# castorini/dhr

Hardware: AMD Instinct MI355X
Metric: queries/sec (exact top-1000, brute-force dense-hybrid GIP retrieval) (higher is better)
Workload: dtype i8 (bound GEMM: gated AND ungated columns int8 x int8 -> int32 on the matrix cores, every gated rounding upward, the ungated quantisation error paid by the filter margin) + f64-accumulated f16 x f32 exact rescoring of the survivors -- the returned scores are the exact scores rounded once, identical

## Files before the change

dhr_amd/csrc/dhr_internal.h:

```cpp
#pragma once
#include <hip/hip_runtime.h>
#include <hip/hip_fp16.h>
#include <stdint.h>

#include "../../include/dhr_hip.h"
#include "abi_guard.h"

extern "C" int dhr_set_error_message(int code, const char* msg);
extern "C" int dhr_index_device(const dhr_index* ix);
extern "C" void dhr_internal_index_arena(dhr_index* ix, void*** base, size_t** bytes);
extern "C" int dhr_internal_search_begin_async(dhr_index* ix, const dhr_query_batch* qb, int32_t k, float* out_sample_scores_dev, void* stream);
extern "C" void dhr_internal_search_abort(dhr_index* ix);
extern "C" int dhr_internal_search_pre_async(dhr_index* ix, const dhr_query_batch* qb, int32_t k, int32_t r_local, float* out_scores_dev, void* stream);
extern "C" int dhr_internal_search_begin_rest_async(dhr_index* ix, const float* tau_dev, float* out_sample_scores_dev, void* stream);
extern "C" int dhr_internal_search_mid_async(dhr_index* ix, const float* tau_hat_dev, int32_t r_local, float* out_scores_dev, void* stream);
extern "C" int dhr_internal_search_finish_async(dhr_index* ix, const float* tau_hat_dev, float* out_scores, int64_t* out_rows, int32_t* out_count_dev,
                                                int32_t out_mem_kind, void* stream);

namespace dhr {

constexpr int TILE_ROWS = 256;
constexpr int TILE_K = 64;
constexpr int CHUNK = 8;
constexpr int TILE_HALVES = TILE_ROWS * TILE_K;
constexpr int SP_A_BYTES = 16384;
constexpr int SP_IDX_BYTES = 2048;
constexpr int SP_STAGE_A = SP_A_BYTES + SP_IDX_BYTES;
constexpr int SP_STAGE_B = 16384;
constexpr int SP_DENSE = 16384;
constexpr int SP_SLOT = SP_STAGE_A + SP_STAGE_B;
constexpr int S8_A_BYTES = 8192;
constexpr int S8_STAGE_A = S8_A_BYTES + 2048;
#ifndef DHR_HEAVY
#define DHR_HEAVY 64
#endif
constexpr int HEAVY = DHR_HEAVY;
constexpr int HEAVY_KEY_STRIDE = HEAVY * 6 / 4;
constexpr int HEAVY_VAL_STRIDE = HEAVY * 6 / 2;
#ifndef DHR_DOC_GROUP
#define DHR_DOC_GROUP 4
#endif
constexpr int DOC_GROUP = DHR_DOC_GROUP;

__host__ __device__ inline int64_t tiled_chunk_offset(int64_t row, int chunk, int ksteps) {
  const int64_t tile = row >> 8;
  const int rl = (int)(row & 255);
  const int ks = chunk >> 3, cc = chunk & 7;
  const int phys = cc ^ ((rl >> 1) & 7);
  return ((tile * ksteps + ks) * TILE_ROWS + rl) * (int64_t)TILE_K + phys * CHUNK;
}

__host__ __device__ inline uint32_t f32_ordered(float f) {
  union { float f; uint32_t u; } v; v.f = f;
  if ((v.u << 1) == 0u) return 0x80000000u;
  return (v.u & 0x80000000u) ? ~v.u : (v.u | 0x80000000u);
}
__host__ __device__ inline float ordered_f32(uint32_t o) {
  union { float f; uint32_t u; } v;
  v.u = (o & 0x80000000u) ? (o & 0x7FFFFFFFu) : ~o;
  return v.f;
}
__host__ __device__ inline int64_t seq_to_tile(int64_t i, int map_mode, int period, int64_t head, int64_t perm_mul = 1, int64_t perm_n = 1) {
  if (map_mode == 0) return i;
  if (map_mode == 1) return head + i * period;
  if (map_mode == 3) i = (i * perm_mul) % perm_n;
  return head + (i / (period - 1)) * period + i % (period - 1) + 1;
}
__host__ __device__ inline int64_t divmod24(int64_t x, int64_t n, double inv_n, int64_t& rem) {
  const double xd = (double)(int32_t)(x >> 24) * 16777216.0 + (double)(int32_t)(x & 0xFFFFFF);
  int64_t q = (int64_t)(int32_t)(xd * inv_n);
  int64_t r = x - q * n;
  if (r < 0) { r += n; --q; } else if (r >= n) { r -= n; ++q; }
  rem = r;
  return q;
}
__host__ __device__ inline int64_t seq_to_tile_fast(int64_t i, int map_mode, int period, int64_t head, int64_t perm_mul, int64_t perm_n,
                                                    double inv_perm_n, double inv_pm1) {
  if (map_mode == 0) return i;
  if (map_mode == 1) return head + i * period;
  if (map_mode == 3) (void)divmod24(i * perm_mul, perm_n, inv_perm_n, i);
  int64_t rem;
  const int64_t q = divmod24(i, period - 1, inv_pm1, rem);
  return head + q * period + rem + 1;
}
__host__ __device__ inline uint64_t make_key(float score, uint32_t row) {
  return ((uint64_t)f32_ordered(score) << 32) | (uint64_t)(0xFFFFFFFFu - row);
}

struct GemmArgs {
  const __half* a_tiles;
  const __half* b_tiles;
  int ksteps;
  int k_split;
  int ts, td;
  int ts_q;
  int64_t seq_lo, seq_hi;
  int map_mode, period;
  int64_t perm_mul, perm_n;
  double inv_perm_n, inv_pm1;
  int64_t head, n_tiles;
  int n_qtiles;
  int64_t n_rows;
  const float* thr;
  uint2* cand;
  uint32_t* cnt;
  uint32_t cap;
  float* dump;
  int64_t dump_ld;
  int64_t dump_row0;
  int n_queries;
  int variant;
  const int32_t* g8_shift;
  const int32_t* g8_rsum;
  int partial_wn;
  uint32_t* p_ctr;
  int64_t p_groups;
  const float* i8_mul;
  const struct ListTier* tier;
};
struct ListTier { uint2* ovf; const uint32_t* ovf_off; const uint32_t* ovf_cap; };
#if defined(__HIPCC__)
// ... 204 lines not shown
```

dhr_amd/csrc/index_build.hip:

```cpp
#include <fcntl.h>
#include <sys/mman.h>
#include <sys/stat.h>
#include <unistd.h>

#include "dhr_state.h"

extern "C" void dhr_index_destroy(dhr_index* ix) try {
  if (!ix) return;
  hipSetDevice(ix->device);
  free_ws(ix->ws);
  free_ws(ix->ws_fb[0]);
  free_ws(ix->ws_fb[1]);
  if (ix->s_aux) hipStreamDestroy(ix->s_aux);
  if (ix->s_gemm) hipStreamDestroy(ix->s_gemm);
  hipFree(ix->sh_arena);
  hipFree(ix->resid8); hipFree(ix->i8_col_scale); hipFree(ix->g8_inv_cs); hipFree(ix->g8_w); hipFree(ix->g8_rsum); hipFree(ix->tiles); hipFree(ix->c_idx); hipFree(ix->vals_rm); hipFree(ix->bucket_map); hipFree(ix->heavy_key);
  delete ix;
} DHR_CATCH_VOID

static int g_opt_dense_i8 = -1;
static int g_opt_gated_i8 = -1;
constexpr int64_t GATED_I8_MIN_ROWS = 1000000, GATED_I8_MIN_ROWS_NARROW = 4000000;
constexpr int64_t DENSE_ONLY_I8_MIN_ROWS = 1000000;
extern "C" int dhr_set_option(int32_t option, int64_t value) try {
// ... 274 lines not shown
        ix->i8_scale = ix->i8_ec = ix->i8_nc = 0.f;
        ix->td = ((d->d_cls + 31) / 32 + 1) & ~1;
        ix->kt = ix->td * 32;
        ix->ksteps = (ix->kt + TILE_K - 1) / TILE_K;
      }
    }
  }
  {
    const int ld = (int)round_up(ix->d_cls, 256) / 2;
    if (ix->dense_i8 && ix->d_dlr == 0 && ld <= 512 && ix->i8_ec > 0.f) {
      const size_t rb = (size_t)ix->n_rows * ld;
      if (hipMalloc((void**)&ix->resid8, rb) != hipSuccess) return fail(set_error(DHR_ERR_HIP, "hipMalloc of the residual image failed"));
      ix->index_bytes += (int64_t)rb;
      ix->resid_ld = ld;
      if (launch_resid_build(ix->vals_rm, ix->k_rm, ix->n_rows, ix->d_dlr, ix->d_cls, ix->i8_col_scale, ix->resid8, ld, s) != hipSuccess)
        return fail(set_error(DHR_ERR_HIP, "residual image launch failed"));
      ix->resid_ec2 = std::sqrt((float)ix->d_cls) * ix->i8_scale / 28.f;
    }
  }
  const size_t tile_bytes = (size_t)ix->n_tiles * ((size_t)ix->ts * (ix->gated_i8 ? S8_STAGE_A : SP_STAGE_A) + (size_t)ix->td * SP_DENSE);
  if (hipMalloc((void**)&ix->tiles, tile_bytes) != hipSuccess)
    return fail(set_error(DHR_ERR_HIP, "hipMalloc of " + std::to_string(tile_bytes) + " bytes for the corpus tiles failed"));
  ix->index_bytes += (int64_t)tile_bytes;
  if (ix->gated_i8) {
    float gmax;
    memcpy(&gmax, &flags[3], 4);
    std::vector<uint32_t> cm((size_t)ix->d_dlr, 0u);
    {
      DevMem cmd;
      uint32_t*& d_cm = (uint32_t*&)cmd.p;
      if (hipMalloc((void**)&d_cm, cm.size() * 4) != hipSuccess || hipMalloc((void**)&ix->g8_inv_cs, cm.size() * 4) != hipSuccess ||
          hipMalloc((void**)&ix->g8_w, cm.size() * 4) != hipSuccess)
        return fail(set_error(DHR_ERR_HIP, "hipMalloc failed"));
      if (hipMemsetAsync(d_cm, 0, cm.size() * 4, s) != hipSuccess ||
          launch_col_absmax(ix->vals_rm, ix->k_rm, ix->n_rows, 0, ix->d_dlr, d_cm, s) != hipSuccess ||
          hipMemcpy(cm.data(), d_cm, cm.size() * 4, hipMemcpyDeviceToHost) != hipSuccess)
        return fail(set_error(DHR_ERR_HIP, "column scan failed"));
    }
    ix->g8_sref = (gmax > 0.f ? gmax : 1.f) * (1.00001f / 127.f);
    std::vector<float> inv(cm.size()), wj(cm.size());
    for (size_t j = 0; j < cm.size(); ++j) {
      float m;
      memcpy(&m, &cm[j], 4);
      const float ratio = m > 0.f ? std::min(m / gmax, 1.f) : 1.f;
      const float f = std::max(std::pow(ratio, 0.75f), 1.f / 1024.f);
      inv[j] = 1.000001f / (ix->g8_sref * f);
      wj[j] = f * 1.000001f;
    }
    if (hipMemcpy(ix->g8_inv_cs, inv.data(), inv.size() * 4, hipMemcpyHostToDevice) != hipSuccess ||
        hipMemcpy(ix->g8_w, wj.data(), wj.size() * 4, hipMemcpyHostToDevice) != hipSuccess)
      return fail(set_error(DHR_ERR_HIP, "hipMemcpy failed"));
    ix->g8_max_shift = 0;
    while (ix->g8_max_shift < 7 && 255.0 * 127.0 * (double)(ix->ts * 32) * (double)(2 << ix->g8_max_shift) <= 1073741824.0) ++ix->g8_max_shift;
    const size_t rb = (size_t)ix->n_tiles * TILE_ROWS * 4;
    if (hipMalloc((void**)&ix->g8_rsum, rb) != hipSuccess) return fail(set_error(DHR_ERR_HIP, "hipMalloc failed"));
    ix->index_bytes += (int64_t)rb;
    if (launch_g8_row_sum(ix->vals_rm, ix->k_rm, ix->n_rows, ix->n_tiles * TILE_ROWS, ix->d_dlr, ix->abs_mode, ix->g8_inv_cs, ix->g8_rsum, s) != hipSuccess)
      return fail(set_error(DHR_ERR_HIP, "g8_row_sum launch failed"));
  }
  if (has_idx && ix->n_buckets == 1) {
    const size_t mb = (size_t)d->d_dlr * 256;
    if (hipMalloc((void**)&ix->bucket_map, mb) != hipSuccess || hipMemsetAsync(ix->bucket_map, 0, mb, s) != hipSuccess)
      return fail(set_error(DHR_ERR_HIP, "bucket map allocation failed"));
  }
  if (has_idx && ix->n_buckets > 1 && idx_esize(d->index_dtype) == 1) {
    const size_t hb = (size_t)d->d_dlr * 256 * 4;
    if (hipMalloc((void**)&d_hist, hb) != hipSuccess || hipMemsetAsync(d_hist, 0, hb, s) != hipSuccess)
      return fail(set_error(DHR_ERR_HIP, "hipMalloc (index histogram) failed"));
    if (launch_idx_hist((const uint8_t*)ix->c_idx, ix->vals_rm, ix->k_rm, d->n_rows, d->d_dlr, (float*)d_hist, s) != hipSuccess)
      return fail(set_error(DHR_ERR_HIP, "idx_hist launch failed"));
    std::vector<float> hist((size_t)d->d_dlr * 256);
    if (hipMemcpy(hist.data(), d_hist, hb, hipMemcpyDeviceToHost) != hipSuccess) return fail(set_error(DHR_ERR_HIP, "hipMemcpy failed"));
    std::vector<uint8_t> map;
    build_bucket_map(hist, d->d_dlr, ix->n_buckets, map);
    if (hipMalloc((void**)&ix->bucket_map, map.size()) != hipSuccess ||
        hipMemcpy(ix->bucket_map, map.data(), map.size(), hipMemcpyHostToDevice) != hipSuccess)
      return fail(set_error(DHR_ERR_HIP, "bucket map upload failed"));
  }
  if ((rc = build_tiles(ix, s)) != DHR_OK) return fail(rc);
  if (has_idx && d->d_dlr <= 4096) {
    const size_t hb = (size_t)d->n_rows * HEAVY_KEY_STRIDE * 4;
    if (hipMalloc((void**)&ix->heavy_key, hb) != hipSuccess)
      return fail(set_error(DHR_ERR_HIP, "hipMalloc of the refine lists failed"));
    ix->heavy_val = (__half*)((char*)ix->heavy_key + HEAVY * 4);
    ix->index_bytes += (int64_t)hb;
    if (launch_heavy_build(ix->vals_rm, ix->k_rm, ix->c_idx, ix->idx_dtype, d->n_rows, d->d_dlr, ix->bucket_map, ix->n_buckets,
                           ix->heavy_key, ix->heavy_val, ix->gated_i8 ? ix->g8_inv_cs : nullptr, ix->abs_mode ? 1 : 0, s) != hipSuccess)
      return fail(set_error(DHR_ERR_HIP, "heavy_build launch failed"));
  }
  if (hipStreamSynchronize(s) != hipSuccess) return fail(set_error(DHR_ERR_HIP, "index build failed on the device"));
  build.ix = nullptr;
  *out = ix;
  return DHR_OK;
} DHR_CATCH_STATUS

namespace {
struct FileHeader {
  char magic[8];
  uint32_t version, header_bytes;
  int64_t n_rows, row_offset;
  int32_t d_dlr, d_cls, k_rm, idx_dtype, idx_buckets, pad0;
  uint64_t val_offset, val_bytes, idx_offset, idx_bytes, blob_offset, blob_bytes;
};
static_assert(sizeof(FileHeader) <= 4096, "header must fit one page");
const char FILE_MAGIC[8] = {'D', 'H', 'R', 'I', 'D', 'X', '1', 0};
constexpr uint32_t FILE_VERSION = 1;

bool write_all(int fd, const void* p, size_t n) {
  const char* c = (const char*)p;
  while (n) {
    const ssize_t w = write(fd, c, n);
    if (w <= 0) return false;
    c += w; n -= (size_t)w;
  }
  return true;
}
int read_header(const char* path, FileHeader& h, int* fd_out) {
  if (!path) return set_error(DHR_ERR_INVALID, "null path");
  const int fd = open(path, O_RDONLY);
  if (fd < 0) return set_error(DHR_ERR_INVALID, std::string("cannot open ") + path);
  char page[4096];
  const ssize_t got = pread(fd, page, sizeof(page), 0);
  if (got != (ssize_t)sizeof(page)) { close(fd); return set_error(DHR_ERR_INVALID, std::string(path) + " is not a device-ready index file (short header)"); }
  memcpy(&h, page, sizeof(h));
  if (memcmp(h.magic, FILE_MAGIC, 8) != 0 || h.header_bytes != 4096) { close(fd); return set_error(DHR_ERR_INVALID, std::string(path) + " is not a device-ready index file"); }
  if (h.version != FILE_VERSION) {
    close(fd);
    return set_error(DHR_ERR_UNSUPPORTED, std::string(path) + " has file format version " + std::to_string(h.version) + ", this library reads version " +
                                          std::to_string(FILE_VERSION));
  }
  if (fd_out) *fd_out = fd; else close(fd);
  return DHR_OK;
}
}

extern "C" int dhr_index_save(const dhr_index* ix, const char* path, const void* blob, int64_t blob_bytes) try {
  if (!ix || !path || blob_bytes < 0 || (blob_bytes > 0 && !blob)) return set_error(DHR_ERR_INVALID, "null index / path or bad blob");
  HIP_TRY(hipSetDevice(ix->device));
  FileHeader h{};
  memcpy(h.magic, FILE_MAGIC, 8);
  h.version = FILE_VERSION; h.header_bytes = 4096;
  h.n_rows = ix->n_rows; h.row_offset = ix->row_offset;
  h.d_dlr = ix->d_dlr; h.d_cls = ix->d_cls; h.k_rm = ix->k_rm; h.idx_dtype = ix->idx_dtype; h.idx_buckets = ix->idx_buckets_req;
  h.pad0 = ix->dlr_pad;
  h.val_offset = 4096; h.val_bytes = (uint64_t)ix->n_rows * ix->k_rm * 2;
  h.idx_offset = (h.val_offset + h.val_bytes + 4095) / 4096 * 4096;
  h.idx_bytes = ix->c_idx ? (uint64_t)ix->n_rows * ix->d_dlr * idx_esize(ix->idx_dtype) : 0;
  h.blob_offset = (h.idx_offset + h.idx_bytes + 4095) / 4096 * 4096;
  h.blob_bytes = (uint64_t)blob_bytes;
  const int fd = open(path, O_WRONLY | O_CREAT | O_TRUNC, 0644);
  if (fd < 0) return set_error(DHR_ERR_INVALID, std::string("cannot create ") + path);
  const size_t CH = (size_t)64 << 20;
  void* pin = nullptr;
  if (hipHostMalloc(&pin, CH, hipHostMallocDefault) != hipSuccess) { close(fd); return set_error(DHR_ERR_HIP, "hipHostMalloc failed"); }
  auto fail = [&](int code) { hipHostFree(pin); close(fd); unlink(path); return code; };
  char page[4096] = {0};
  memcpy(page, &h, sizeof(h));
  if (!write_all(fd, page, 4096)) return fail(set_error(DHR_ERR_INVALID, "write failed (header)"));
  const void* src[2] = {ix->vals_rm, ix->c_idx};
  const uint64_t off[2] = {h.val_offset, h.idx_offset}, bytes[2] = {h.val_bytes, h.idx_bytes};
  for (int i = 0; i < 2; ++i) {
    if (lseek(fd, (off_t)off[i], SEEK_SET) < 0) return fail(set_error(DHR_ERR_INVALID, "seek failed"));
    for (uint64_t done = 0; done < bytes[i]; done += CH) {
      const size_t n = (size_t)std::min<uint64_t>(CH, bytes[i] - done);
      if (hipMemcpy(pin, (const char*)src[i] + done, n, hipMemcpyDeviceToHost) != hipSuccess) return fail(set_error(DHR_ERR_HIP, "D2H copy failed while saving"));
      if (!write_all(fd, pin, n)) return fail(set_error(DHR_ERR_INVALID, "write failed (disk full?)"));
    }
// ... 54 lines not shown
```

dhr_amd/csrc/kernels.hip:

```cpp
#include <algorithm>
#include <cstdlib>
#include <mutex>

#include "dhr_internal.h"
#include "gemm_common.h"
#include <type_traits>

namespace dhr {

typedef short short8 __attribute__((ext_vector_type(8)));

static hipError_t ensure_lds_attr(const void* fn, int bytes, int (&have)[64]) {
  static std::mutex mu;
  int dev = 0;
  (void)hipGetDevice(&dev);
  std::lock_guard<std::mutex> lock(mu);
  if (bytes <= have[dev & 63]) return hipSuccess;
  const hipError_t e = hipFuncSetAttribute(fn, hipFuncAttributeMaxDynamicSharedMemorySize, bytes);
  if (e == hipSuccess) have[dev & 63] = bytes;
  return e;
}

__device__ __forceinline__ float wave_sum(float v) {
#pragma unroll
// ... 668 lines not shown
  __syncthreads();
  for (int d = 512; d > 0; d >>= 1) {
    if (tid < d) part[tid] += part[tid + d];
    __syncthreads();
  }
  if (tid == 0) {
    const unsigned long long total = part[0] + 256ull * (unsigned long long)n_queries;
    scale_s = total > arena_entries ? (double)arena_entries / (double)total : 1.0;
  }
  __syncthreads();
  const double scale = scale_s;
  auto seg = [&](int q) -> uint32_t {
    const uint32_t w = want(q);
    if (w == 0u) return 0u;
    const uint32_t v = scale < 1.0 ? (uint32_t)((double)w * scale) : w;
    return (v + 255u) & ~255u;
  };
  __syncthreads();
  s = 0;
  for (int q = lo; q < hi; ++q) s += seg(q);
  part[tid] = s;
  __syncthreads();
  for (int d = 1; d < 1024; d <<= 1) {
    const unsigned long long v = tid >= d ? part[tid - d] : 0ull;
    __syncthreads();
    part[tid] += v;
    __syncthreads();
  }
  unsigned long long run = tid ? part[tid - 1] : 0ull;
  for (int q = lo; q < hi; ++q) {
    uint32_t w = seg(q);
    if (run >= arena_entries) w = 0u;
    else if (run + w > arena_entries) w = (uint32_t)(arena_entries - run);
    ovf_off[q] = (uint32_t)(run < arena_entries ? run : arena_entries);
    ovf_cap[q] = w;
    run += seg(q);
  }
}
hipError_t launch_plan_overflow(const uint32_t* cnt_prev, double rows_ratio, uint32_t cap, uint32_t max_extra, uint32_t arena_entries, int n_queries,
                                uint32_t* ovf_off, uint32_t* ovf_cap, hipStream_t s) {
  hipLaunchKernelGGL(plan_overflow_kernel, dim3(1), dim3(1024), 0, s, cnt_prev, rows_ratio, cap, max_extra, arena_entries, n_queries, ovf_off, ovf_cap);
  return hipGetLastError();
}
__device__ __forceinline__ bool flat_block(const uint32_t* __restrict__ offs, int n_queries, uint32_t b, int& q, uint32_t& blk) {
  if (b >= offs[n_queries]) return false;
  int lo = 0, hi = n_queries;
  while (hi - lo > 1) {
    const int mid = (lo + hi) >> 1;
    if (offs[mid] <= b) lo = mid; else hi = mid;
  }
  q = lo; blk = b - offs[lo];
  return true;
}

template <int SL>
__global__ void __launch_bounds__(256) heavy_build_kernel(const __half* __restrict__ vals_rm, int k_rm,
                                                          const void* __restrict__ idx, int idx_dtype, int64_t n_rows,
                                                          int d_dlr, const uint8_t* __restrict__ map, int n_buckets,
                                                          uint32_t* __restrict__ heavy_key, __half* __restrict__ heavy_val,
                                                          const float* __restrict__ g8_inv_cs, int abs_mode) {
  const int lane = threadIdx.x & 63;
  const int64_t wave0 = (int64_t)blockIdx.x * 4 + (threadIdx.x >> 6);
  const int64_t nwaves = (int64_t)gridDim.x * 4;
  for (int64_t row = wave0; row < n_rows; row += nwaves) {
    constexpr int MAXJ = 64 * SL - 1;
    uint32_t key[SL];
#pragma unroll
    for (int sl = 0; sl < SL; ++sl) {
      const int j = lane + 64 * sl;
      key[sl] = 0u;
      if (j < d_dlr) {
        union { _Float16 h; uint16_t u; } cv; cv.h = (_Float16)__half2float(vals_rm[row * k_rm + j]);
        const uint32_t mag = cv.u & 0x7FFFu;
        if (mag) key[sl] = (mag << 16) | (uint32_t)(MAXJ - j);
      }
    }
    for (int r = 0; r < HEAVY; ++r) {
      uint32_t best = 0u;
#pragma unroll
      for (int sl = 0; sl < SL; ++sl) best = key[sl] > best ? key[sl] : best;
#pragma unroll
      for (int o = 32; o > 0; o >>= 1) { const uint32_t ob = __shfl_xor(best, o, 64); best = ob > best ? ob : best; }
      if (best == 0u) {
        if (lane == 0) for (int rr = r; rr < HEAVY; ++rr) { heavy_key[row * HEAVY_KEY_STRIDE + rr] = 0xFFFFFFFFu; heavy_val[row * HEAVY_VAL_STRIDE + rr] = __float2half(0.f); }
        break;
      }
      const int j = MAXJ - (int)(best & 0xFFFFu);
      if ((j & 63) == lane) {
        const int iv = load_idx(idx, idx_dtype, row * d_dlr + j);
        const uint32_t bk = n_buckets > 1 ? (uint32_t)bucket_of(iv, j, map, n_buckets) : 0u;
        uint32_t key_out = ((uint32_t)j << 20) | (bk << 16) | ((uint32_t)iv & 0xFFFFu);
        if (g8_inv_cs) {
          float d = __half2float(vals_rm[row * k_rm + j]);
          if (abs_mode) d = fabsf(d);
          const uint32_t lvl = d > 0.f ? (uint32_t)quant_up_i8(d, g8_inv_cs[j]) : 0u;
          key_out = ((uint32_t)j << 20) | ((lvl >> 4) << 17) | ((bk & 1u) << 16) | ((lvl & 0xFu) << 12) | ((uint32_t)iv & 0xFFFu);
        }
        heavy_key[row * HEAVY_KEY_STRIDE + r] = key_out;
        heavy_val[row * HEAVY_VAL_STRIDE + r] = vals_rm[row * k_rm + j];
#pragma unroll
        for (int sl = 0; sl < SL; ++sl) if (sl == (j >> 6)) key[sl] = 0u;
      }
    }
  }
}
hipError_t launch_heavy_build(const __half* vals_rm, int k_rm, const void* idx, int idx_dtype, int64_t n_rows, int d_dlr,
                              const uint8_t* map, int n_buckets, uint32_t* heavy_key, __half* heavy_val, const float* g8_inv_cs, int abs_mode, hipStream_t s) {
  if (n_rows <= 0) return hipSuccess;
  const int64_t blocks = (n_rows + 3) / 4;
  if (d_dlr <= 1024)
    hipLaunchKernelGGL(heavy_build_kernel<16>, dim3((unsigned)(blocks < 16384 ? blocks : 16384)), dim3(256), 0, s, vals_rm, k_rm,
                       idx, idx_dtype, n_rows, d_dlr, map, n_buckets, heavy_key, heavy_val, g8_inv_cs, abs_mode);
  else
    hipLaunchKernelGGL(heavy_build_kernel<64>, dim3((unsigned)(blocks < 16384 ? blocks : 16384)), dim3(256), 0, s, vals_rm, k_rm,
                       idx, idx_dtype, n_rows, d_dlr, map, n_buckets, heavy_key, heavy_val, g8_inv_cs, abs_mode);
  return hipGetLastError();
}

static __device__ __forceinline__ uint4 gather16(const void* p) { return *(const uint4*)p; }
static __device__ __forceinline__ uint2 gather8(const void* p) { return *(const uint2*)p; }
#ifndef REFINE_PREFETCH
#define REFINE_PREFETCH 2
#endif
#ifndef REFINE_WPE
#define REFINE_WPE 8
#endif
#if REFINE_WPE > 0
#define REFINE_ATTR __attribute__((amdgpu_waves_per_eu(REFINE_WPE)))
#else
#define REFINE_ATTR
#endif
template <bool G8>
__global__ void __launch_bounds__(256) REFINE_ATTR refine_kernel(RefineArgs p) {
  extern __shared__ uint32_t qw[];
  int q = blockIdx.y;
  uint32_t blk = blockIdx.x;
  for (uint32_t fb = blockIdx.x;; fb += gridDim.x) {
  if (p.blk_off && !flat_block(p.blk_off, p.n_queries, fb, q, blk)) return;
  uint32_t count = p.cnt[q];
  const uint32_t cap_q = p.ovf_cap ? p.cap + p.ovf_cap[q] : p.cap;
  if (count > cap_q) count = cap_q;
  const uint32_t base = blk * REFINE_PER_WG;
  if (base >= count) { if (p.blk_off) continue; return; }
  __syncthreads();
  for (int j = threadIdx.x; j < p.d_dlr; j += 256) {
    if constexpr (G8) { qw[2 * j] = p.q_pack[(int64_t)q * p.d_dlr + j]; qw[2 * j + 1] = p.g8_q8[(int64_t)q * p.d_dlr + j]; }
    else qw[j] = p.q_pack[(int64_t)q * p.d_dlr + j];
  }
  __syncthreads();
  const int sub = threadIdx.x & 7;
  const float t = p.thr[q];
  const double unit = G8 ? (double)p.g8_unit[q] : 0.0;
  auto entry = [&](uint32_t i) __attribute__((always_inline)) -> uint2 {
    if (i >= count || i >= base + REFINE_PER_WG) return make_uint2(0u, 0u);
    return i < p.cap ? p.cand[(int64_t)q * p.cap + i] : p.ovf[(size_t)p.ovf_off[q] + (i - p.cap)];
  };
  constexpr int EPL = HEAVY / 8;
  static_assert(EPL == 8 || EPL == 4, "8 lanes per candidate read 8 or 4 entries each");
  struct Rec { uint4 k0, k1, hv; };
  auto record = [&](uint32_t i, const uint2 c, Rec& r) __attribute__((always_inline)) {
    r.k0 = r.k1 = make_uint4(0xFFFFFFFFu, 0xFFFFFFFFu, 0xFFFFFFFFu, 0xFFFFFFFFu);
    r.hv = make_uint4(0u, 0u, 0u, 0u);
    if (i < count && i < base + REFINE_PER_WG) {
      const uint32_t* hk = p.heavy_key + (int64_t)c.x * HEAVY_KEY_STRIDE + sub * EPL;
      r.k0 = gather16(hk);
      if constexpr (EPL == 8) {
        r.k1 = gather16(hk + 4);
        r.hv = gather16(p.heavy_val + (int64_t)c.x * HEAVY_VAL_STRIDE + sub * 8);
      } else {
        const uint2 v2 = gather8(p.heavy_val + (int64_t)c.x * HEAVY_VAL_STRIDE + sub * 4);
        r.hv = make_uint4(v2.x, v2.y, 0u, 0u);
      }
    }
  };
  const uint32_t i_first = base + (threadIdx.x >> 3);
#if REFINE_PREFETCH >= 1
  uint2 c_cur = entry(i_first), c_nx = entry(i_first + 32);
#endif
#if REFINE_PREFETCH >= 2
  Rec r_cur;
  record(i_first, c_cur, r_cur);
#endif
  for (uint32_t i = i_first; i < base + REFINE_PER_WG; i += 32) {
    float corr = 0.f;
    int taken = 0;
    double back = 0.0;
#if REFINE_PREFETCH >= 2
    const uint2 c = c_cur;
    const Rec rc = r_cur;
    Rec r_nx;
    record(i + 32, c_nx, r_nx);
    const uint2 c_nx2 = entry(i + 64);
    c_cur = c_nx; c_nx = c_nx2; r_cur = r_nx;
#elif REFINE_PREFETCH == 1
    const uint2 c = c_cur;
    c_cur = c_nx; c_nx = entry(i + 64);
    Rec rc;
    record(i, c, rc);
#else
    const uint2 c = entry(i);
    Rec rc;
    record(i, c, rc);
#endif
    if (i < count) {
      const uint4 k0 = rc.k0, k1 = rc.k1;
      union { uint4 u; half8 h; } hvu;
      hvu.u = rc.hv;
      const half8 hv = hvu.h;
      const uint32_t keys[8] = {k0.x, k0.y, k0.z, k0.w, k1.x, k1.y, k1.z, k1.w};
#pragma unroll
      for (int e = 0; e < EPL; ++e) {
        const uint32_t key = keys[e];
        if (key != 0xFFFFFFFFu) {
          const uint32_t j = key >> 20;
          if constexpr (G8) {
            const uint2 wq = *(const uint2*)(qw + 2 * j);
            const uint32_t w = wq.x;
            const bool same_bucket = p.ungated || ((w >> 12) & 0x1u) == ((key >> 16) & 0x1u);
            const bool mismatch = !p.ungated && (w & 0xFFFu) != (key & 0xFFFu);
            const int lvl = (int)(((key >> 17) & 0x7u) << 4 | ((key >> 12) & 0xFu));
            if (same_bucket && lvl > 0) {
              taken += (int)wq.y * lvl;
              if (!mismatch) {
                union { uint16_t u; _Float16 h; } qv; qv.u = (uint16_t)(w >> 16);
                const float d = p.abs_mode ? fabsf((float)hv[e]) : (float)hv[e];
                back += (double)(float)qv.h * (double)d;
              }
            }
          } else {
            const uint32_t w = qw[j];
            const bool same_bucket = ((w >> 12) & 0xFu) == ((key >> 16) & 0xFu);
            const bool mismatch = (w & 0xFFFu) != (key & 0xFFFu);
            union { uint16_t u; _Float16 h; } qv; qv.u = (uint16_t)(w >> 16);
            if (same_bucket && mismatch) corr += fabsf((float)qv.h * (float)hv[e]);
          }
        }
      }
    }
    if constexpr (G8) {
      taken += __shfl_xor(taken, 1, 64); taken += __shfl_xor(taken, 2, 64); taken += __shfl_xor(taken, 4, 64);
      back += __shfl_xor(back, 1, 64); back += __shfl_xor(back, 2, 64); back += __shfl_xor(back, 4, 64);
    } else {
      corr += __shfl_xor(corr, 1, 64);
      corr += __shfl_xor(corr, 2, 64);
      corr += __shfl_xor(corr, 4, 64);
    }
    if (sub == 0 && i < count) {
      float u2;
      if constexpr (G8) {
        const double v = (double)__uint_as_float(c.y) - (double)taken * unit + back;
        u2 = (float)v;
        if ((double)u2 < v) u2 = nextafterf(u2, INFINITY);
      } else u2 = __uint_as_float(c.y) - corr;
      if (u2 >= t) {
        const uint32_t slot = atomicAdd(p.out_cnt + q, 1u);
        if (slot < p.out_cap) p.out[(int64_t)q * p.out_cap + slot] = make_uint2(c.x, __float_as_uint(u2));
      }
    }
  }
  if (!p.blk_off) return;
  }
}
__global__ void __launch_bounds__(256) resid_build_kernel(const __half* __restrict__ vals_rm, int k_rm, int64_t n_rows, int d_dlr, int d_cls,
                                                          const float* __restrict__ col_scale, uint8_t* __restrict__ resid8, int ld) {
  const int64_t total = n_rows * (ld / 8);
  for (int64_t g = (int64_t)blockIdx.x * blockDim.x + threadIdx.x; g < total; g += (int64_t)gridDim.x * blockDim.x) {
    const int64_t row = g / (ld / 8);
    const int c0 = (int)(g - row * (ld / 8)) * 16;
    uint32_t w[2] = {0u, 0u};
#pragma unroll
    for (int e = 0; e < 16; ++e) {
      const int c = c0 + e;
      int r4 = 0;
      if (c < d_cls) {
        const float cs = col_scale[c];
        const float f = __half2float(vals_rm[row * k_rm + d_dlr + c]);
        const float rho = f - cs * (float)quant_i8(f, 1.f / cs);
        float t = rintf(rho * (14.f / cs));
        t = t < -7.f ? -7.f : (t > 7.f ? 7.f : t);
        r4 = (int)t;
      }
      w[e >> 3] |= (uint32_t)(r4 + 8) << (4 * (e & 7));
    }
    *(uint2*)(resid8 + row * ld + c0 / 2) = make_uint2(w[0], w[1]);
  }
}
hipError_t launch_resid_build(const __half* vals_rm, int k_rm, int64_t n_rows, int d_dlr, int d_cls, const float* col_scale, uint8_t* resid8, int resid_ld, hipStream_t s) {
  if (n_rows <= 0) return hipSuccess;
  const int64_t blocks = (n_rows * (resid_ld / 8) + 255) / 256;
  hipLaunchKernelGGL(resid_build_kernel, dim3((unsigned)(blocks < 65536 ? blocks : 65536)), dim3(256), 0, s, vals_rm, k_rm, n_rows, d_dlr, d_cls, col_scale, resid8, resid_ld);
  return hipGetLastError();
}
#ifndef DENSE_REFINE_WPE
#define DENSE_REFINE_WPE 8
#endif
#if DENSE_REFINE_WPE > 0
#define DENSE_REFINE_ATTR __attribute__((amdgpu_waves_per_eu(DENSE_REFINE_WPE)))
#else
#define DENSE_REFINE_ATTR
#endif
#ifndef DENSE_REFINE_LPC
#define DENSE_REFINE_LPC 16
#endif
template <int CH>
__global__ void __launch_bounds__(256) DENSE_REFINE_ATTR dense_refine_kernel(RefineArgs p) {
  constexpr int LPC = DENSE_REFINE_LPC, PB = 128 / LPC, WPP = PB / 4;
  static_assert(LPC == 16 || LPC == 8, "one load instruction of a candidate's lanes = one 128-byte line");
  __shared__ float a_s[1024];
  __shared__ uint32_t f_s[2 * 128];
  __shared__ float red[3 * 4];
  int q = blockIdx.y;
  uint32_t blk = blockIdx.x;
  const int sub = threadIdx.x & (LPC - 1), lane = threadIdx.x & 63, wave = threadIdx.x >> 6;
  constexpr int NCOL = CH * 16;
  for (uint32_t fb = blockIdx.x;; fb += gridDim.x) {
  if (p.blk_off && !flat_block(p.blk_off, p.n_queries, fb, q, blk)) return;
  uint32_t count = p.cnt[q];
  const uint32_t cap_q = p.ovf_cap ? p.cap + p.ovf_cap[q] : p.cap;
  if (count > cap_q) count = cap_q;
  const uint32_t base = blk * REFINE_PER_WG;
  if (base >= count) { if (p.blk_off) continue; return; }
  __syncthreads();
  float mx = 0.f;
  for (int j = threadIdx.x; j < NCOL; j += 256) {
    const float a = j < p.d_cls ? p.q32[(int64_t)q * p.q32_ld + j] * p.col_scale[j] * (1.f / 14.f) : 0.f;
    a_s[j] = a;
    mx = fmaxf(mx, fabsf(a));
  }
#pragma unroll
  for (int o = 32; o > 0; o >>= 1) mx = fmaxf(mx, __shfl_xor(mx, o, 64));
  if (lane == 0) red[wave] = mx;
  __syncthreads();
  mx = fmaxf(fmaxf(red[0], red[1]), fmaxf(red[2], red[3]));
  const float sa = mx > 0.f && mx < INFINITY ? mx * (1.f / 127.f) : 1.f, inv_sa = 1.f / sa;
  float s8 = 0.f, sd = 0.f;
  for (int g8 = threadIdx.x; g8 < NCOL / 8; g8 += 256) {
// ... 1150 lines not shown
```

Baseline: 58250.

## Split refine into two-stage heavy-entry pass with early candidate rejection

Rearranges each row's heavy refine list so the top 20 entries (keys and values) sit in a compact interleaved first block and the remaining 44 in a second block. The refine kernel first scores every candidate with 4 lanes over only those 20 entries. It then compacts the survivors per wave into shared memory and reads the remaining entries only for them. The aim is to avoid reading and processing most of the heavy list for candidates that the partial bound already rules out. The cost is extra shared-memory staging, a ballot-based compaction step and a changed on-disk/device layout, which needs all builders and readers to agree.

Result: faster. 59760 (median of 6 runs) (+2.6%).

```diff
diff --git a/dhr_amd/csrc/dhr_internal.h b/dhr_amd/csrc/dhr_internal.h
--- a/dhr_amd/csrc/dhr_internal.h
+++ b/dhr_amd/csrc/dhr_internal.h
@@ -31,12 +31,21 @@
 constexpr int SP_SLOT = SP_STAGE_A + SP_STAGE_B;
 constexpr int S8_A_BYTES = 8192;
 constexpr int S8_STAGE_A = S8_A_BYTES + 2048;
-#ifndef DHR_HEAVY
-#define DHR_HEAVY 64
-#endif
-constexpr int HEAVY = DHR_HEAVY;
+constexpr int HEAVY = 64;
+constexpr int HEAVY_B0 = 20;
 constexpr int HEAVY_KEY_STRIDE = HEAVY * 6 / 4;
 constexpr int HEAVY_VAL_STRIDE = HEAVY * 6 / 2;
+__host__ __device__ inline int heavy_key_word(int r) {
+  if (r < HEAVY_B0) return 8 * (r / 5) + r % 5;
+  r -= HEAVY_B0;
+  return 32 + 16 * (r / 11) + r % 11;
+}
+__host__ __device__ inline int heavy_val_half(int r) {
+  if (r < HEAVY_B0) return 2 * (8 * (r / 5) + 5) + r % 5;
+  r -= HEAVY_B0;
+  const int s = r / 11, e = r % 11;
+  return e < 10 ? 2 * (32 + 16 * s + 11) + e : 2 * (8 * s + 5) + 5;
+}
 #ifndef DHR_DOC_GROUP
 #define DHR_DOC_GROUP 4
 #endif
diff --git a/dhr_amd/csrc/index_build.hip b/dhr_amd/csrc/index_build.hip
--- a/dhr_amd/csrc/index_build.hip
+++ b/dhr_amd/csrc/index_build.hip
@@ -380,7 +380,7 @@
     const size_t hb = (size_t)d->n_rows * HEAVY_KEY_STRIDE * 4;
     if (hipMalloc((void**)&ix->heavy_key, hb) != hipSuccess)
       return fail(set_error(DHR_ERR_HIP, "hipMalloc of the refine lists failed"));
-    ix->heavy_val = (__half*)((char*)ix->heavy_key + HEAVY * 4);
+    ix->heavy_val = (__half*)ix->heavy_key;
     ix->index_bytes += (int64_t)hb;
     if (launch_heavy_build(ix->vals_rm, ix->k_rm, ix->c_idx, ix->idx_dtype, d->n_rows, d->d_dlr, ix->bucket_map, ix->n_buckets,
                            ix->heavy_key, ix->heavy_val, ix->gated_i8 ? ix->g8_inv_cs : nullptr, ix->abs_mode ? 1 : 0, s) != hipSuccess)
diff --git a/dhr_amd/csrc/kernels.hip b/dhr_amd/csrc/kernels.hip
--- a/dhr_amd/csrc/kernels.hip
+++ b/dhr_amd/csrc/kernels.hip
@@ -774,7 +774,7 @@
 #pragma unroll
       for (int o = 32; o > 0; o >>= 1) { const uint32_t ob = __shfl_xor(best, o, 64); best = ob > best ? ob : best; }
       if (best == 0u) {
-        if (lane == 0) for (int rr = r; rr < HEAVY; ++rr) { heavy_key[row * HEAVY_KEY_STRIDE + rr] = 0xFFFFFFFFu; heavy_val[row * HEAVY_VAL_STRIDE + rr] = __float2half(0.f); }
+        if (lane == 0) for (int rr = r; rr < HEAVY; ++rr) { heavy_key[row * HEAVY_KEY_STRIDE + heavy_key_word(rr)] = 0xFFFFFFFFu; heavy_val[row * HEAVY_VAL_STRIDE + heavy_val_half(rr)] = __float2half(0.f); }
         break;
       }
       const int j = MAXJ - (int)(best & 0xFFFFu);
@@ -788,8 +788,8 @@
           const uint32_t lvl = d > 0.f ? (uint32_t)quant_up_i8(d, g8_inv_cs[j]) : 0u;
           key_out = ((uint32_t)j << 20) | ((lvl >> 4) << 17) | ((bk & 1u) << 16) | ((lvl & 0xFu) << 12) | ((uint32_t)iv & 0xFFFu);
         }
-        heavy_key[row * HEAVY_KEY_STRIDE + r] = key_out;
-        heavy_val[row * HEAVY_VAL_STRIDE + r] = vals_rm[row * k_rm + j];
+        heavy_key[row * HEAVY_KEY_STRIDE + heavy_key_word(r)] = key_out;
+        heavy_val[row * HEAVY_VAL_STRIDE + heavy_val_half(r)] = vals_rm[row * k_rm + j];
 #pragma unroll
         for (int sl = 0; sl < SL; ++sl) if (sl == (j >> 6)) key[sl] = 0u;
       }
@@ -813,6 +813,9 @@
 static __device__ __forceinline__ uint2 gather8(const void* p) { return *(const uint2*)p; }
 #ifndef REFINE_PREFETCH
 #define REFINE_PREFETCH 2
+#endif
+#ifndef REFINE_L2_PREFETCH
+#define REFINE_L2_PREFETCH 0
 #endif
 #ifndef REFINE_WPE
 #define REFINE_WPE 8
@@ -824,9 +827,17 @@
 #endif
 template <bool G8>
 __global__ void __launch_bounds__(256) REFINE_ATTR refine_kernel(RefineArgs p) {
+  static_assert(REFINE_PER_WG % 64 == 0 && HEAVY_B0 == 20 && HEAVY == 64, "4 lanes x 5 entries, then 4 lanes x 11 entries per candidate; 64 candidates per round");
   extern __shared__ uint32_t qw[];
+  constexpr int WSLOTS = REFINE_PER_WG / 4;
+  __shared__ uint2 sv_c[REFINE_PER_WG];
+  __shared__ uint32_t sv_t[REFINE_PER_WG];
+  __shared__ double sv_b[G8 ? REFINE_PER_WG : 1];
+  __shared__ uint16_t sv_s[REFINE_PER_WG * 4];
   int q = blockIdx.y;
   uint32_t blk = blockIdx.x;
+  const int sub = threadIdx.x & 3, lane = threadIdx.x & 63;
+  const uint32_t slot0 = (threadIdx.x >> 6) * WSLOTS;
   for (uint32_t fb = blockIdx.x;; fb += gridDim.x) {
   if (p.blk_off && !flat_block(p.blk_off, p.n_queries, fb, q, blk)) return;
   uint32_t count = p.cnt[q];
@@ -840,110 +851,174 @@
     else qw[j] = p.q_pack[(int64_t)q * p.d_dlr + j];
   }
   __syncthreads();
-  const int sub = threadIdx.x & 7;
   const float t = p.thr[q];
   const double unit = G8 ? (double)p.g8_unit[q] : 0.0;
+  const uint32_t end = base + REFINE_PER_WG;
+  auto look = [&](const uint32_t key, const uint32_t hbits, int& taken, double& back, float& corr) __attribute__((always_inline)) {
+    if (key == 0xFFFFFFFFu) return;
+    const uint32_t j = key >> 20;
+    union { uint16_t u; _Float16 h; } dv; dv.u = (uint16_t)hbits;
+    if constexpr (G8) {
+      const uint2 wq = *(const uint2*)(qw + 2 * j);
+      const uint32_t w = wq.x;
+      const bool same_bucket = p.ungated || ((w >> 12) & 0x1u) == ((key >> 16) & 0x1u);
+      const bool mismatch = !p.ungated && (w & 0xFFFu) != (key & 0xFFFu);
+      const int lvl = (int)(((key >> 17) & 0x7u) << 4 | ((key >> 12) & 0xFu));
+      if (same_bucket && lvl > 0) {
+        taken += (int)wq.y * lvl;
+        if (!mismatch) {
+          union { uint16_t u; _Float16 h; } qv; qv.u = (uint16_t)(w >> 16);
+          const float d = p.abs_mode ? fabsf((float)dv.h) : (float)dv.h;
+          back += (double)(float)qv.h * (double)d;
+        }
+      }
+    } else {
+      const uint32_t w = qw[j];
+      const bool same_bucket = ((w >> 12) & 0xFu) == ((key >> 16) & 0xFu);
+      const bool mismatch = (w & 0xFFFu) != (key & 0xFFFu);
+      union { uint16_t u; _Float16 h; } qv; qv.u = (uint16_t)(w >> 16);
+      if (same_bucket && mismatch) corr += fabsf((float)qv.h * (float)dv.h);
+    }
+  };
+  auto bound_g8 = [&](const uint32_t u_bits, const int taken, const double back) __attribute__((always_inline)) -> float {
+    const double v = (double)__uint_as_float(u_bits) - (double)taken * unit + back;
+    float u2 = (float)v;
+    if ((double)u2 < v) u2 = nextafterf(u2, INFINITY);
+    return u2;
+  };
   auto entry = [&](uint32_t i) __attribute__((always_inline)) -> uint2 {
-    if (i >= count || i >= base + REFINE_PER_WG) return make_uint2(0u, 0u);
+    if (i >= count || i >= end) return make_uint2(0u, 0u);
     return i < p.cap ? p.cand[(int64_t)q * p.cap + i] : p.ovf[(size_t)p.ovf_off[q] + (i - p.cap)];
   };
-  constexpr int EPL = HEAVY / 8;
-  static_assert(EPL == 8 || EPL == 4, "8 lanes per candidate read 8 or 4 entries each");
-  struct Rec { uint4 k0, k1, hv; };
-  auto record = [&](uint32_t i, const uint2 c, Rec& r) __attribute__((always_inline)) {
-    r.k0 = r.k1 = make_uint4(0xFFFFFFFFu, 0xFFFFFFFFu, 0xFFFFFFFFu, 0xFFFFFFFFu);
-    r.hv = make_uint4(0u, 0u, 0u, 0u);
-    if (i < count && i < base + REFINE_PER_WG) {
-      const uint32_t* hk = p.heavy_key + (int64_t)c.x * HEAVY_KEY_STRIDE + sub * EPL;
-      r.k0 = gather16(hk);
-      if constexpr (EPL == 8) {
-        r.k1 = gather16(hk + 4);
-        r.hv = gather16(p.heavy_val + (int64_t)c.x * HEAVY_VAL_STRIDE + sub * 8);
-      } else {
-        const uint2 v2 = gather8(p.heavy_val + (int64_t)c.x * HEAVY_VAL_STRIDE + sub * 4);
-        r.hv = make_uint4(v2.x, v2.y, 0u, 0u);
-      }
+  struct Rec1 { uint4 a, b; };
+  auto record1 = [&](uint32_t i, const uint2 c, Rec1& r) __attribute__((always_inline)) {
+    r.a = make_uint4(0xFFFFFFFFu, 0xFFFFFFFFu, 0xFFFFFFFFu, 0xFFFFFFFFu);
+    r.b = make_uint4(0xFFFFFFFFu, 0u, 0u, 0u);
+    if (i < count && i < end) {
+      const uint32_t* h = p.heavy_key + (int64_t)c.x * HEAVY_KEY_STRIDE + sub * 8;
+      r.a = gather16(h);
+      r.b = gather16(h + 4);
     }
   };
-  const uint32_t i_first = base + (threadIdx.x >> 3);
+  uint32_t n_w = 0;
+  const uint32_t i_first = base + (threadIdx.x >> 2);
 #if REFINE_PREFETCH >= 1
-  uint2 c_cur = entry(i_first), c_nx = entry(i_first + 32);
+  uint2 c_cur = entry(i_first), c_nx = entry(i_first + 64);
 #endif
 #if REFINE_PREFETCH >= 2
-  Rec r_cur;
-  record(i_first, c_cur, r_cur);
+  Rec1 r_cur;
+  record1(i_first, c_cur, r_cur);
 #endif
-  for (uint32_t i = i_first; i < base + REFINE_PER_WG; i += 32) {
+  for (uint32_t i = i_first; i < end; i += 64) {
+#if REFINE_PREFETCH >= 2
+    const uint2 c = c_cur;
+    const Rec1 rc = r_cur;
+    Rec1 r_nx;
+    record1(i + 64, c_nx, r_nx);
+    const uint2 c_nx2 = entry(i + 128);
+    c_cur = c_nx; c_nx = c_nx2; r_cur = r_nx;
+#elif REFINE_PREFETCH == 1
+    const uint2 c = c_cur;
+    c_cur = c_nx; c_nx = entry(i + 128);
+    Rec1 rc;
+    record1(i, c, rc);
+#else
+    const uint2 c = entry(i);
+    Rec1 rc;
+    record1(i, c, rc);
+#endif
     float corr = 0.f;
     int taken = 0;
     double back = 0.0;
-#if REFINE_PREFETCH >= 2
-    const uint2 c = c_cur;
-    const Rec rc = r_cur;
-    Rec r_nx;
-    record(i + 32, c_nx, r_nx);
-    const uint2 c_nx2 = entry(i + 64);
-    c_cur = c_nx; c_nx = c_nx2; r_cur = r_nx;
-#elif REFINE_PREFETCH == 1
-    const uint2 c = c_cur;
-    c_cur = c_nx; c_nx = entry(i + 64);
-    Rec rc;
-    record(i, c, rc);
-#else
-    const uint2 c = entry(i);
-    Rec rc;
-    record(i, c, rc);
-#endif
-    if (i < count) {
-      const uint4 k0 = rc.k0, k1 = rc.k1;
-      union { uint4 u; half8 h; } hvu;
-      hvu.u = rc.hv;
-      const half8 hv = hvu.h;
-      const uint32_t keys[8] = {k0.x, k0.y, k0.z, k0.w, k1.x, k1.y, k1.z, k1.w};
-#pragma unroll
-      for (int e = 0; e < EPL; ++e) {
-        const uint32_t key = keys[e];
-        if (key != 0xFFFFFFFFu) {
-          const uint32_t j = key >> 20;
-          if constexpr (G8) {
-            const uint2 wq = *(const uint2*)(qw + 2 * j);
-            const uint32_t w = wq.x;
-            const bool same_bucket = p.ungated || ((w >> 12) & 0x1u) == ((key >> 16) & 0x1u);
-            const bool mismatch = !p.ungated && (w & 0xFFFu) != (key & 0xFFFu);
-            const int lvl = (int)(((key >> 17) & 0x7u) << 4 | ((key >> 12) & 0xFu));
-            if (same_bucket && lvl > 0) {
-              taken += (int)wq.y * lvl;
-              if (!mismatch) {
-                union { uint16_t u; _Float16 h; } qv; qv.u = (uint16_t)(w >> 16);
-                const float d = p.abs_mode ? fabsf((float)hv[e]) : (float)hv[e];
-                back += (double)(float)qv.h * (double)d;
-              }
-            }
-          } else {
-            const uint32_t w = qw[j];
-            const bool same_bucket = ((w >> 12) & 0xFu) == ((key >> 16) & 0xFu);
-            const bool mismatch = (w & 0xFFFu) != (key & 0xFFFu);
-            union { uint16_t u; _Float16 h; } qv; qv.u = (uint16_t)(w >> 16);
-            if (same_bucket && mismatch) corr += fabsf((float)qv.h * (float)hv[e]);
-          }
-        }
-      }
+    const bool valid = i < count;
+    if (valid) {
+      look(rc.a.x, rc.b.y & 0xFFFFu, taken, back, corr);
+      look(rc.a.y, rc.b.y >> 16, taken, back, corr);
+      look(rc.a.z, rc.b.z & 0xFFFFu, taken, back, corr);
+      look(rc.a.w, rc.b.z >> 16, taken, back, corr);
+      look(rc.b.x, rc.b.w & 0xFFFFu, taken, back, corr);
     }
     if constexpr (G8) {
-      taken += __shfl_xor(taken, 1, 64); taken += __shfl_xor(taken, 2, 64); taken += __shfl_xor(taken, 4, 64);
-      back += __shfl_xor(back, 1, 64); back += __shfl_xor(back, 2, 64); back += __shfl_xor(back, 4, 64);
+      taken += __shfl_xor(taken, 1, 64); taken += __shfl_xor(taken, 2, 64);
+      back += __shfl_xor(back, 1, 64); back += __shfl_xor(back, 2, 64);
     } else {
       corr += __shfl_xor(corr, 1, 64);
       corr += __shfl_xor(corr, 2, 64);
-      corr += __shfl_xor(corr, 4, 64);
-    }
-    if (sub == 0 && i < count) {
+    }
+    bool keep = false;
+    if (valid) {
+      if constexpr (G8) keep = nextafterf(bound_g8(c.y, taken, back), INFINITY) >= t;
+      else keep = __uint_as_float(c.y) - corr >= t;
+    }
+    const unsigned long long m = __ballot(keep);
+    if (keep) {
+      const uint32_t slot = slot0 + n_w + (uint32_t)__popcll(m & ((1ull << (lane & ~3)) - 1ull)) / 4u;
+      sv_s[slot * 4 + sub] = (uint16_t)(rc.b.w >> 16);
+      if (sub == 0) {
+        sv_c[slot] = c;
+        if constexpr (G8) { sv_t[slot] = (uint32_t)taken; sv_b[slot] = back; }
+        else sv_t[slot] = __float_as_uint(corr);
+      }
+    }
+    n_w += (uint32_t)__popcll(m) / 4u;
+  }
+  __syncthreads();
+  n_w = (uint32_t)__builtin_amdgcn_readfirstlane((int)n_w);
+  struct Rec2 { uint4 a, b, c, d; };
+  auto record2 = [&](uint32_t k, Rec2& r) __attribute__((always_inline)) {
+    r.a = r.b = make_uint4(0xFFFFFFFFu, 0xFFFFFFFFu, 0xFFFFFFFFu, 0xFFFFFFFFu);
+    r.c = make_uint4(0xFFFFFFFFu, 0xFFFFFFFFu, 0xFFFFFFFFu, 0u);
+    r.d = make_uint4(0u, 0u, 0u, 0u);
+    if (k < n_w) {
+      const uint32_t* h = p.heavy_key + (int64_t)sv_c[slot0 + k].x * HEAVY_KEY_STRIDE + 32 + sub * 16;
+      r.a = gather16(h);
+      r.b = gather16(h + 4);
+      r.c = gather16(h + 8);
+      r.d = gather16(h + 12);
+    }
+  };
+#if REFINE_L2_PREFETCH
+  Rec2 s_cur;
+  record2((uint32_t)(lane >> 2), s_cur);
+#endif
+  for (uint32_t k0 = 0; k0 < n_w; k0 += 16) {
+    const uint32_t k = k0 + (uint32_t)(lane >> 2);
+#if REFINE_L2_PREFETCH
+    const Rec2 rc = s_cur;
+    record2(k + 16, s_cur);
+#else
+    Rec2 rc;
+    record2(k, rc);
+#endif
+    float corr = 0.f;
+    int taken = 0;
+    double back = 0.0;
+    const bool valid = k < n_w;
+    if (valid) {
+      look(rc.a.x, rc.c.w & 0xFFFFu, taken, back, corr);
+      look(rc.a.y, rc.c.w >> 16, taken, back, corr);
+      look(rc.a.z, rc.d.x & 0xFFFFu, taken, back, corr);
+      look(rc.a.w, rc.d.x >> 16, taken, back, corr);
+      look(rc.b.x, rc.d.y & 0xFFFFu, taken, back, corr);
+      look(rc.b.y, rc.d.y >> 16, taken, back, corr);
+      look(rc.b.z, rc.d.z & 0xFFFFu, taken, back, corr);
+      look(rc.b.w, rc.d.z >> 16, taken, back, corr);
+      look(rc.c.x, rc.d.w & 0xFFFFu, taken, back, corr);
+      look(rc.c.y, rc.d.w >> 16, taken, back, corr);
+      look(rc.c.z, (uint32_t)sv_s[(slot0 + k) * 4 + sub], taken, back, corr);
+    }
+    if constexpr (G8) {
+      taken += __shfl_xor(taken, 1, 64); taken += __shfl_xor(taken, 2, 64);
+      back += __shfl_xor(back, 1, 64); back += __shfl_xor(back, 2, 64);
+    } else {
+      corr += __shfl_xor(corr, 1, 64);
+      corr += __shfl_xor(corr, 2, 64);
+    }
+    if (sub == 0 && valid) {
+      const uint2 c = sv_c[slot0 + k];
       float u2;
-      if constexpr (G8) {
-        const double v = (double)__uint_as_float(c.y) - (double)taken * unit + back;
-        u2 = (float)v;
-        if ((double)u2 < v) u2 = nextafterf(u2, INFINITY);
-      } else u2 = __uint_as_float(c.y) - corr;
+      if constexpr (G8) u2 = bound_g8(c.y, (int)sv_t[slot0 + k] + taken, sv_b[slot0 + k] + back);
+      else u2 = __uint_as_float(c.y) - (__uint_as_float(sv_t[slot0 + k]) + corr);
       if (u2 >= t) {
         const uint32_t slot = atomicAdd(p.out_cnt + q, 1u);
         if (slot < p.out_cap) p.out[(int64_t)q * p.out_cap + slot] = make_uint2(c.x, __float_as_uint(u2));
```
